# yshen47/SGAM_NeurIPS22

Measured on AMD Instinct MI355X. Metric: generated RGB-D frames/sec (256x256, GoogleEarth), higher is better.
Workload: dtype f32; 1 GPU; GoogleEarth-Infinite 256x256 inference loop (BASELINE configs[2]): forward-splat warp (N<=3) + VQGAN encode/quantise(4096)/decode + frame feedback, in-HBM frame store; frames_per_gpu=1110, scenes=1, parallelism=scene-parallel x1, launch=hip-graph replay of the VQGAN forward, f32_products=exact hi/lo fp16 split on the fp16 matrix cores, fp32 accumulate

## Files before the change

### include/sgam_hip.h

```cpp
#ifndef SGAM_HIP_H
#define SGAM_HIP_H

#include <stdint.h>

#ifdef __cplusplus
extern "C" {
#endif

#define SGAM_OK 0
#define SGAM_EINVAL (-1)
#define SGAM_EALIGN (-2)
#define SGAM_EWORKSPACE (-3)

int sgam_abi_version(void);
const char *sgam_build_info(void);
const char *sgam_build_commit(void);
const char *sgam_build_digest(void);

int sgam_prof_enable(int32_t on);
int sgam_prof_mark_empty(void *stream);
int32_t sgam_prof_count(void);
int sgam_prof_get(int32_t i, const char **kernel, const char **where, float *ms, double *flops, double *bytes);
int sgam_prof_get_shape(int32_t i, int32_t *mnks);

// ... 134 lines not shown
int64_t sgam_attn_block_f32x_workspace_bytes(int32_t n, int32_t C, int32_t B);
int sgam_attn_block_f32x(const float *x, int32_t ldx, const float *mean_rstd, const float *gamma, const float *beta, const void *wqkv_planes,
                         float wqkv_scale, const float *bqkv, int32_t n, int32_t C, int32_t B, float scale, const void *wp_planes,
                         float wp_scale, const float *bp, float *out, int32_t ldc, double *gn_partial, void *workspace,
                         int64_t workspace_bytes, void *stream);
int32_t sgam_attention_small_f32x_fits(int32_t n, int32_t C, int32_t B);
int sgam_attention_small_f32x(const float *q, const float *k, const float *v, int32_t ld, int32_t n, int32_t C, int32_t B, float scale,
                              float *out, int32_t ldo, void *stream);
int sgam_attention_small_h16(const void *q, const void *k, const void *v, int32_t ht, int32_t ld, int32_t n, int32_t C, int32_t B, float scale,
                             void *out, int32_t ldo, void *stream);
int sgam_groupnorm_table_from_partials(const double *partial, int32_t nchunk, const float *gamma, const float *beta,
                                       float *scale_shift, int32_t B, int32_t HW, int32_t C, int32_t groups, float eps, void *stream);
int sgam_pack_qkv_weight_h16(const float *w, void *w_frag, int32_t ht, int32_t C, void *stream);
int sgam_pack_weight_tp_h16(const float *w, void *w_frag, int32_t ht, int32_t rows, int32_t C, void *stream);
int sgam_attn_block_proj_h16(const void *x, int32_t ldx, const double *gn_partial, int32_t nchunk, const float *gamma, const float *beta,
                             float eps, const void *w_frag, const float *bias, int32_t ht, int32_t n, int32_t C, int32_t B, float scale,
                             const void *wp_frag, const float *bp, double *gn_partial_out, void *out, int32_t ldo, void *workspace,
                             int64_t workspace_bytes, void *stream);
int64_t sgam_attn_block_h16_workspace_bytes(int32_t n, int32_t C, int32_t B);
int sgam_attn_block_h16(const void *x, int32_t ldx, const double *gn_partial, int32_t nchunk, const float *gamma, const float *beta,
                        float eps, const void *w_frag, const float *bias, int32_t ht, int32_t n, int32_t C, int32_t B, float scale,
                        void *out, int32_t ldo, void *workspace, int64_t workspace_bytes, void *stream);

int sgam_row_sumsq_f32(const float *x, float *out, int32_t rows, int32_t cols, void *stream);
int64_t sgam_vq_workspace_bytes(int32_t T, int32_t D, int32_t n_e);
int sgam_vq_nearest_f32(const float *z, const float *codebook, const float *e_sq, float *dots,
                        int64_t *idx_out, float *zq_out, float *dist_out, int32_t T, int32_t D,
                        int32_t n_e, int32_t straight_through, void *workspace, int64_t workspace_bytes,
                        void *stream);
int sgam_vq_commit_loss_f32(const float *z, const float *codebook, const int64_t *idx, double *partial, float *loss,
                            int32_t T, int32_t D, int32_t n_e, float beta, void *stream);
int sgam_vq_gather_f32(const float *codebook, const int64_t *idx, float *out, int32_t T, int32_t D,
                       int32_t n_e, void *stream);
int sgam_vq_topk_f32(const float *dist, float *vals, int64_t *inds, int32_t T, int32_t n_e, int32_t k,
                     void *stream);
int sgam_vq_sample_topk_f32(const float *dist, const float *codebook, const uint8_t *mask, const int32_t *stream_id,
                            const uint64_t *call, uint64_t seed, float *vals, int64_t *inds, int64_t *idx_out,
                            float *zq_out, int32_t B, int32_t S, int32_t h, int32_t w, int32_t D, int32_t n_e,
                            int32_t k, int32_t mask_h, int32_t mask_w, int32_t per_token, float temperature,
                            void *stream);

int sgam_nchw_to_nhwc_f32(const float *x, float *y, int32_t B, int32_t C, int32_t HW, int32_t ldy,
                          void *stream);
int sgam_nhwc_to_nchw_f32(const float *x, float *y, int32_t B, int32_t C, int32_t HW, int32_t ldx,
                          void *stream);
int sgam_encode_head_f32(const float *x, const uint8_t *mask, const float *w, const float *bias,
                         float *y, int32_t B, int32_t HW, int32_t ldy, void *stream);

int sgam_forward_splat_f32(const float *src_feats, int64_t feat_cs, int64_t feat_ps,
                           const float *src_depths, const float *tgt_K, const float *src_Kinv,
                           const float *T, int32_t B, int32_t N, int32_t H, int32_t W,
                           const float *depth_range, int32_t dataset_norm, int32_t *winner,
                           float *merge_depths, float *merge_feats, uint8_t *extrap, float *x_out,
                           float *proj_feats, float *proj_depth, uint8_t *inb_mask, int32_t *pix_xy,
                           void *stream);
int sgam_forward_splat_srcs_f32(const float *const *src_feat_ptrs, const float *const *src_depth_ptrs, int64_t feat_cs,
                                int64_t feat_ps, const float *tgt_K, const float *src_Kinv, const float *T, int32_t B,
                                int32_t N, int32_t H, int32_t W, const float *depth_range, int32_t dataset_norm,
                                int32_t *winner, float *merge_depths, float *merge_feats, uint8_t *extrap, float *x_out,
                                float *proj_feats, float *proj_depth, uint8_t *inb_mask, int32_t *pix_xy, void *stream);

int64_t sgam_forward_splat_workspace_bytes(int32_t B, int32_t N, int32_t H, int32_t W);
int64_t sgam_forward_splat_workspace_zero_bytes(int32_t B, int32_t N, int32_t H, int32_t W);
int sgam_forward_splat_tiled_f32(const float *src_feats, int64_t feat_cs, int64_t feat_ps, const float *src_depths,
                                 const float *tgt_K, const float *src_Kinv, const float *T, int32_t B, int32_t N, int32_t H,
                                 int32_t W, const float *depth_range, int32_t dataset_norm, void *workspace,
// ... 142 lines not shown
```

### sgam_neurips22_amd/_lib.py

```python
import ctypes
import os

_PKG = os.path.dirname(os.path.abspath(__file__))
LIB_PATH = os.environ.get("SGAM_HIP_LIB") or os.path.join(_PKG, "lib", "libsgam_hip.so")

c_i32, c_i64, c_f32, c_vp = ctypes.c_int32, ctypes.c_int64, ctypes.c_float, ctypes.c_void_p


class ConvDesc(ctypes.Structure):
    _fields_ = [(n, c_i32) for n in (
        "B", "Hi", "Wi", "Cin", "Ho", "Wo", "N", "KH", "KW", "stride", "pad_t", "pad_l", "upsample2x",
        "lda", "ldb", "ldc", "ldr", "n_valid", "bias_per_row", "plan_bm", "plan_bn", "plan_ksplit")]


class TsdfGrid(ctypes.Structure):
    _fields_ = [("voxel_length", c_f32), ("sdf_trunc", c_f32), ("unit_base", c_i32 * 3), ("unit_dims", c_i32 * 3)]


class TsdfSrc(ctypes.Structure):
    _fields_ = [("depth", c_vp), ("rgb_u8", c_vp), ("cam2world", c_f32 * 16), ("world2cam", c_f32 * 16)]


ABI_VERSION = 10

# ... 129 lines not shown
                                              c_vp]),
    "sgam_softmax_rows_f32": (c_i32, [c_vp, c_i32, c_i32, c_i32, c_f32, c_vp]),
    "sgam_softmax_rows_blockdiag_f32": (c_i32, [c_vp, c_i32, c_i32, c_i32, c_f32, c_i32, c_vp]),
    "sgam_attention_f32x_workspace_bytes": (c_i64, [c_i32, c_i32]),
    "sgam_attention_f32x": (c_i32, [c_vp, c_vp, c_vp, c_i32, c_i32, c_i32, c_f32, c_vp, c_i32, c_vp, c_i64, c_vp]),
    "sgam_attention_h16_workspace_bytes": (c_i64, [c_i32, c_i32]),
    "sgam_attention_h16": (c_i32, [c_vp, c_vp, c_vp, c_i32, c_i32, c_i32, c_i32, c_f32, c_vp, c_i32, c_vp, c_i64, c_vp]),
    "sgam_attention_f32x_batched_workspace_bytes": (c_i64, [c_i32, c_i32, c_i32]),
    "sgam_attention_f32x_batched": (c_i32, [c_vp, c_vp, c_vp, c_i32, c_i32, c_i32, c_i32, c_f32, c_vp, c_i32, c_vp, c_i64, c_vp]),
    "sgam_attention_proj_f32x_batched": (c_i32, [c_vp, c_vp, c_vp, c_i32, c_i32, c_i32, c_i32, c_f32, c_vp, c_f32, c_vp, c_vp, c_i32, c_vp,
                                                 c_i32, c_vp, c_vp, c_i64, c_vp]),
    "sgam_attention_h16_batched_workspace_bytes": (c_i64, [c_i32, c_i32, c_i32]),
    "sgam_attention_h16_batched": (c_i32, [c_vp, c_vp, c_vp, c_i32, c_i32, c_i32, c_i32, c_i32, c_f32, c_vp, c_i32, c_vp, c_i64, c_vp]),
    "sgam_attn_block_f32x_workspace_bytes": (c_i64, [c_i32, c_i32, c_i32]),
    "sgam_attn_block_f32x": (c_i32, [c_vp, c_i32, c_vp, c_vp, c_vp, c_vp, c_f32, c_vp, c_i32, c_i32, c_i32, c_f32, c_vp, c_f32, c_vp, c_vp, c_i32,
                                     c_vp, c_vp, c_i64, c_vp]),
    "sgam_attention_small_f32x_fits": (c_i32, [c_i32, c_i32, c_i32]),
    "sgam_attention_small_f32x": (c_i32, [c_vp, c_vp, c_vp, c_i32, c_i32, c_i32, c_i32, c_f32, c_vp, c_i32, c_vp]),
    "sgam_attention_small_h16": (c_i32, [c_vp, c_vp, c_vp, c_i32, c_i32, c_i32, c_i32, c_i32, c_f32, c_vp, c_i32, c_vp]),
    "sgam_groupnorm_table_from_partials": (c_i32, [c_vp, c_i32, c_vp, c_vp, c_vp, c_i32, c_i32, c_i32, c_i32, c_f32, c_vp]),
    "sgam_pack_qkv_weight_h16": (c_i32, [c_vp, c_vp, c_i32, c_i32, c_vp]),
    "sgam_pack_weight_tp_h16": (c_i32, [c_vp, c_vp, c_i32, c_i32, c_i32, c_vp]),
    "sgam_attn_block_proj_h16": (c_i32, [c_vp, c_i32, c_vp, c_i32, c_vp, c_vp, c_f32, c_vp, c_vp, c_i32, c_i32, c_i32, c_i32, c_f32, c_vp, c_vp,
                                         c_vp, c_vp, c_i32, c_vp, c_i64, c_vp]),
    "sgam_attn_block_h16_workspace_bytes": (c_i64, [c_i32, c_i32, c_i32]),
    "sgam_attn_block_h16": (c_i32, [c_vp, c_i32, c_vp, c_i32, c_vp, c_vp, c_f32, c_vp, c_vp, c_i32, c_i32, c_i32, c_i32, c_f32, c_vp, c_i32,
                                    c_vp, c_i64, c_vp]),
    "sgam_row_sumsq_f32": (c_i32, [c_vp, c_vp, c_i32, c_i32, c_vp]),
    "sgam_vq_workspace_bytes": (c_i64, [c_i32, c_i32, c_i32]),
    "sgam_vq_nearest_f32": (c_i32, [c_vp, c_vp, c_vp, c_vp, c_vp, c_vp, c_vp, c_i32, c_i32, c_i32, c_i32, c_vp,
                                    c_i64, c_vp]),
    "sgam_vq_commit_loss_f32": (c_i32, [c_vp, c_vp, c_vp, c_vp, c_vp, c_i32, c_i32, c_i32, c_f32, c_vp]),
    "sgam_vq_gather_f32": (c_i32, [c_vp, c_vp, c_vp, c_i32, c_i32, c_i32, c_vp]),
    "sgam_vq_topk_f32": (c_i32, [c_vp, c_vp, c_vp, c_i32, c_i32, c_i32, c_vp]),
    "sgam_vq_sample_topk_f32": (c_i32, [c_vp, c_vp, c_vp, c_vp, c_vp, ctypes.c_uint64, c_vp, c_vp, c_vp, c_vp, c_i32, c_i32, c_i32, c_i32,
                                        c_i32, c_i32, c_i32, c_i32, c_i32, c_i32, c_f32, c_vp]),
    "sgam_nchw_to_nhwc_f32": (c_i32, [c_vp, c_vp, c_i32, c_i32, c_i32, c_i32, c_vp]),
    "sgam_nhwc_to_nchw_f32": (c_i32, [c_vp, c_vp, c_i32, c_i32, c_i32, c_i32, c_vp]),
    "sgam_encode_head_f32": (c_i32, [c_vp, c_vp, c_vp, c_vp, c_vp, c_i32, c_i32, c_i32, c_vp]),
    "sgam_forward_splat_f32": (c_i32, [c_vp, c_i64, c_i64, c_vp, c_vp, c_vp, c_vp, c_i32, c_i32, c_i32, c_i32,
                                       ctypes.POINTER(c_f32), c_i32, c_vp, c_vp, c_vp, c_vp, c_vp, c_vp, c_vp,
                                       c_vp, c_vp, c_vp]),
    "sgam_forward_splat_srcs_f32": (c_i32, [c_vp, c_vp, c_i64, c_i64, c_vp, c_vp, c_vp, c_i32, c_i32, c_i32, c_i32,
                                            ctypes.POINTER(c_f32), c_i32, c_vp, c_vp, c_vp, c_vp, c_vp, c_vp, c_vp,
                                            c_vp, c_vp, c_vp]),
    "sgam_forward_splat_workspace_bytes": (c_i64, [c_i32, c_i32, c_i32, c_i32]),
    "sgam_forward_splat_workspace_zero_bytes": (c_i64, [c_i32, c_i32, c_i32, c_i32]),
    "sgam_forward_splat_tiled_f32": (c_i32, [c_vp, c_i64, c_i64, c_vp, c_vp, c_vp, c_vp, c_i32, c_i32, c_i32, c_i32,
                                             ctypes.POINTER(c_f32), c_i32, c_vp, c_i64, c_vp, c_vp, c_vp, c_vp, c_vp, c_vp, c_vp]),
    "sgam_forward_splat_tiled_srcs_f32": (c_i32, [c_vp, c_vp, c_i64, c_i64, c_vp, c_vp, c_vp, c_i32, c_i32, c_i32, c_i32,
                                                  ctypes.POINTER(c_f32), c_i32, c_vp, c_i64, c_vp, c_vp, c_vp, c_vp, c_vp, c_vp,
                                                  c_vp]),
    "sgam_depth_normalise_f32": (c_i32, [c_vp, c_i32, c_vp, c_vp, c_i32, c_i64, c_vp]),
    "sgam_inverse_warp_f32": (c_i32, [c_vp, c_vp, c_vp, c_vp, c_vp, c_vp, c_i32, c_i32, c_i32, c_i32, c_vp, c_vp,
                                      c_vp]),
    "sgam_inverse_warp_srcs_f32": (c_i32, [c_vp, c_vp, c_i64, c_i64, c_vp, c_vp, c_vp, c_vp, c_i32, c_i32, c_i32, c_i32,
                                           c_vp, c_vp, c_vp]),
    "sgam_rgb_u8_to_f32": (c_i32, [c_vp, c_vp, c_vp, c_i64, c_vp]),
    "sgam_frame_feedback_f32": (c_i32, [c_vp, c_vp, c_i32, c_vp, c_vp, c_vp, c_i32, c_i32, c_vp]),
    "sgam_resize_lanczos_u8": (c_i32, [c_vp, c_i32, c_i32, c_i32, c_i32, c_i32, c_vp, c_vp, c_vp, c_i32, c_vp, c_vp, c_vp, c_i32,
                                       c_vp, c_vp, c_vp, c_vp]),
    "sgam_resize_nearest_f32": (c_i32, [c_vp, c_i32, c_i32, c_i32, c_i32, c_i32, c_vp, c_i32, c_f32, c_f32, c_vp, c_vp]),
}

_ERRORS = {-1: "SGAM_EINVAL (bad shape / unsupported size)", -2: "SGAM_EALIGN (pointer/stride alignment)",
           -3: "SGAM_EWORKSPACE (workspace missing or too small)"}
# ... 35 lines not shown
```

### sgam_neurips22_amd/csrc/vq.hip

```cpp
#include "sgam_common.h"

namespace {

__device__ __forceinline__ void argmin_combine(float &d, int &j, float od, int oj) {
    if (od < d || (od == d && oj < j)) {
        d = od;
        j = oj;
    }
}

__global__ __launch_bounds__(256) void vq_argmin_kernel(const float *__restrict__ z, const float *__restrict__ codebook,
                                                        const float *__restrict__ e_sq, const float *__restrict__ dots,
                                                        int64_t *__restrict__ idx_out, float *__restrict__ zq_out,
                                                        float *__restrict__ dist_out, int D, int n_e,
                                                        int straight_through) {
    const int t = blockIdx.x;
    const float *zr = z + (int64_t)t * D;
    __shared__ float red_f[4];
    __shared__ int red_i[4];
    __shared__ float bc_f;
    __shared__ int bc_i;

    float zz = 0.f;
    for (int c = threadIdx.x; c < D; c += 256) zz = __fmaf_rn(zr[c], zr[c], zz);
// ... 183 lines not shown
                                                                int T, int D, int n_e) {
    const int t = blockIdx.x * 4 + (threadIdx.x >> 6);
    if (t >= T) return;
    const int lane = threadIdx.x & 63;
    int64_t j = idx[t];
    j = j < 0 ? 0 : (j >= n_e ? n_e - 1 : j);
    double s = 0.0;
    for (int c = lane; c < D; c += 64) {
        const float d = __fsub_rn(codebook[j * D + c], z[(int64_t)t * D + c]);
        s += (double)d * (double)d;
    }
#pragma unroll
    for (int o = 32; o > 0; o >>= 1) s += __shfl_xor(s, o, 64);
    if (lane == 0) partial[t] = s;
}

__global__ __launch_bounds__(256) void vq_commit_fold_kernel(const double *__restrict__ partial, float *__restrict__ loss,
                                                             int T, int D, float beta) {
    __shared__ double red[256];
    double s = 0.0;
    for (int t = threadIdx.x; t < T; t += 256) s += partial[t];
    red[threadIdx.x] = s;
    __syncthreads();
    for (int o = 128; o > 0; o >>= 1) {
        if ((int)threadIdx.x < o) red[threadIdx.x] += red[threadIdx.x + o];
        __syncthreads();
    }
    if (threadIdx.x == 0) {
        const float m = (float)(red[0] / ((double)T * (double)D));
        loss[0] = __fadd_rn(m, __fmul_rn(beta, m));
    }
}

}

extern "C" int sgam_vq_commit_loss_f32(const float *z, const float *codebook, const int64_t *idx, double *partial,
                                       float *loss, int32_t T, int32_t D, int32_t n_e, float beta, void *stream) {
    if (!z || !codebook || !idx || !partial || !loss || T <= 0 || D <= 0 || n_e <= 0) return SGAM_EINVAL;
    SGAM_KLAUNCH(vq_commit_partial_kernel, dim3(sgam_cdiv(T, 4)), dim3(256), 0, sgam_stream(stream), z, codebook, idx,
                       partial, T, D, n_e);
    SGAM_LAUNCH_CHECK();
    SGAM_KLAUNCH(vq_commit_fold_kernel, dim3(1), dim3(256), 0, sgam_stream(stream), partial, loss, T, D, beta);
    SGAM_LAUNCH_CHECK();
    return SGAM_OK;
}

extern "C" int sgam_row_sumsq_f32(const float *x, float *out, int32_t rows, int32_t cols, void *stream) {
    if (!x || !out || rows <= 0 || cols <= 0) return SGAM_EINVAL;
    SGAM_KLAUNCH(row_sumsq_kernel, dim3(sgam_cdiv(rows, 4)), dim3(256), 0, sgam_stream(stream), x, out, rows, cols);
    SGAM_LAUNCH_CHECK();
    return SGAM_OK;
}

static sgam_conv_desc vq_dot_desc(int32_t T, int32_t D, int32_t n_e) {
    sgam_conv_desc d = {};
    d.B = 1; d.Hi = 1; d.Wi = T; d.Cin = D; d.Ho = 1; d.Wo = T; d.N = n_e;
    d.KH = 1; d.KW = 1; d.stride = 1; d.pad_t = 0; d.pad_l = 0; d.upsample2x = 0;
    d.lda = D; d.ldb = D; d.ldc = n_e; d.ldr = 0; d.n_valid = n_e; d.bias_per_row = 0;
    return d;
}

extern "C" int64_t sgam_vq_workspace_bytes(int32_t T, int32_t D, int32_t n_e) {
    if (T <= 0 || D <= 0 || D % 32 != 0 || n_e <= 0 || n_e % 64 != 0) return -1;
    const sgam_conv_desc d = vq_dot_desc(T, D, n_e);
    return sgam_conv2d_workspace_bytes(&d);
}
// ... 20 lines not shown
    SGAM_KLAUNCH(vq_gather_kernel, dim3(sgam_cdiv(total, 256)), dim3(256), 0, sgam_stream(stream), codebook, idx,
                       out, T, D, n_e);
    SGAM_LAUNCH_CHECK();
    return SGAM_OK;
}

extern "C" int sgam_vq_topk_f32(const float *dist, float *vals, int64_t *inds, int32_t T, int32_t n_e, int32_t k,
                                void *stream) {
    if (!dist || !vals || !inds || T <= 0 || n_e <= 0 || k <= 0 || k > 64 || k > n_e) return SGAM_EINVAL;
    SGAM_KLAUNCH(vq_topk_kernel, dim3(T), dim3(256), 0, sgam_stream(stream), dist, vals, inds, n_e, k);
    SGAM_LAUNCH_CHECK();
    return SGAM_OK;
}

extern "C" int sgam_vq_sample_topk_f32(const float *dist, const float *codebook, const uint8_t *mask, const int32_t *stream_id,
                                       const uint64_t *call, uint64_t seed, float *vals, int64_t *inds, int64_t *idx_out,
                                       float *zq_out, int32_t B, int32_t S, int32_t h, int32_t w, int32_t D, int32_t n_e,
                                       int32_t k, int32_t mask_h, int32_t mask_w, int32_t per_token, float temperature,
                                       void *stream) {
    if (!dist || !codebook || !stream_id || !call || !vals || !inds || !idx_out || !zq_out) return SGAM_EINVAL;
    if (B <= 0 || S <= 0 || h <= 0 || w <= 0 || D <= 0 || D % 4 != 0 || n_e <= 0 || k <= 0 || k > 32 || k > n_e) return SGAM_EINVAL;
    if (mask && (mask_h <= 0 || mask_w <= 0)) return SGAM_EINVAL;
    if (!(temperature > 0.f)) return SGAM_EINVAL;
    const int64_t T = (int64_t)h * w, rows = (int64_t)B * T, items = rows * S;
    if (rows > 0x7fffffff || items > 0x7fffffff || T * S > 0x7fffffff) return SGAM_EINVAL;
    SGAM_KLAUNCH(vq_topk_kernel, dim3((unsigned)rows), dim3(256), 0, sgam_stream(stream), dist, vals, inds, n_e, k);
    SGAM_LAUNCH_CHECK();
    SGAM_KLAUNCH(vq_sample_topk_kernel, dim3((unsigned)sgam_cdiv(items, 4)), dim3(256), 0, sgam_stream(stream), vals, inds,
                 codebook, mask, stream_id, reinterpret_cast<const uint32_t *>(call), (uint32_t)(seed & 0xffffffffu),
                 (uint32_t)(seed >> 32), idx_out, zq_out, B, S, h, w, D, n_e, k, mask_h, mask_w, per_token, temperature);
    SGAM_LAUNCH_CHECK();
    return SGAM_OK;
}
```

### sgam_neurips22_amd/generative_sensing_module/model.py

```python
import torch
import torch.nn as nn

from .. import ops
from ..point_rendering.warp import splat_to_model_input
from .modules.diffusionmodules.model import Conv2d, Decoder, Encoder
from .modules.vqvae.quantize import VectorQuantizer2 as VectorQuantizer


class VQModel(nn.Module):
    global_step = 0
    global_rank = 0

    def __init__(self, ddconfig, data_config, lossconfig, n_embed, embed_dim, phase=None, ckpt_path=None,
                 ignore_keys=['loss.discriminator'], image_key="image", colorize_nlabels=None, logdir=None,
                 use_extrapolation_mask=True, vq_step_threshold=0, monitor=None, remap=None, sane_index_shape=False,
                 online_kmeans_config=None, batch_size=None, depth_range=None):
        super().__init__()
        online_kmeans_config = online_kmeans_config or {}
        self.phase = phase
        self.online_kmeans_config = online_kmeans_config
        self.data_config = data_config
        self.logdir = logdir
        self.depth_range = depth_range
        self.n_embed = n_embed
# ... 96 lines not shown
        return _cm()

    def _forward_graphed(self, input, topk, extrapolation_mask, sample_number, flags):
        inplace = getattr(input, "_sgam_persistent", False) and (
            extrapolation_mask is None or getattr(extrapolation_mask, "_sgam_persistent", False))
        if self.compute_dtype == torch.float32 and ops.F32_MODE == "split":
            ops.range_flag(input.device)
        key = (tuple(input.shape), None if extrapolation_mask is None else tuple(extrapolation_mask.shape), topk,
               sample_number, flags, self.compute_dtype, str(input.device), ops.RANGE_FLAG_EPOCH,
               (input.data_ptr(), None if extrapolation_mask is None else extrapolation_mask.data_ptr()) if inplace else None)
        ent = self._graphs.get(key)
        if ent is None:
            sx = input if inplace else input.detach().clone()
            sm = None if extrapolation_mask is None else (extrapolation_mask if inplace else extrapolation_mask.detach().clone())
            side = torch.cuda.Stream()
            side.wait_stream(torch.cuda.current_stream())
            with torch.cuda.stream(side):
                for _ in range(2):
                    self._forward_guarded(sx, topk, sm, sample_number, flags)
            torch.cuda.current_stream().wait_stream(side)
            graph = torch.cuda.CUDAGraph()
            with torch.cuda.graph(graph):
                out = self._forward_eager(sx, topk, sm, sample_number, *flags)
            ent = self._graphs[key] = (graph, sx, sm, out)
        graph, sx, sm, out = ent
        if not inplace:
            sx.copy_(input)
            if sm is not None:
                sm.copy_(extrapolation_mask)
        graph.replay()
        return out

    def _encode_nhwc(self, x, extrapolation_mask):
        dt = self.compute_dtype
        if self.use_extrapolation_mask:
            h = ops.encode_head(x, extrapolation_mask, self.conv_in.weight, self.conv_in.bias, ld=32, dtype=dt)
        else:
            h = ops.cast(ops.nchw_to_nhwc(x, c_pad=32), dt)
        return self.quant_conv.forward_nhwc(self.encoder.forward_nhwc(h), out_dtype=torch.float32)

    def _decode_nhwc(self, quant_nhwc):
        q = ops.cast(quant_nhwc, self.compute_dtype)
        return self.decoder.forward_nhwc(self.post_quant_conv.forward_nhwc(q))

    def encode(self, x, topk=None, encoding_indices=None, extrapolation_mask=None, use_old=False, sample_number=1):
        pre = self._encode_nhwc(x, extrapolation_mask)
        if not self.use_vq():
            return ops.nhwc_to_nchw(pre)
        if topk is None:
            if encoding_indices is None:
                zq, idx, _ = self.quantize.quantize_nhwc(pre)
            else:
                B, h, w, D = pre.shape
                idx = encoding_indices.reshape(B, h, w)
                zq = ops.vq_gather(self.quantize._codebook()[0], idx).view(B, h, w, D)
            return ops.nhwc_to_nchw(zq), self.quantize.commit_loss_nhwc(pre, idx), (None, None, idx), ops.nhwc_to_nchw(pre)
        zqs, idx = self.quantize.sample_nhwc(pre, topk, sample_number, extrapolation_mask)
        quants = torch.stack([ops.nhwc_to_nchw(zqs[:, i].contiguous()) for i in range(zqs.shape[1])], 1)
        return quants, None, (None, None, idx), ops.nhwc_to_nchw(pre)

    def decode(self, quant):
        return ops.nhwc_to_nchw(self._decode_nhwc(ops.nchw_to_nhwc(quant)))

    def forward(self, input, topk=None, extrapolation_mask=None, sample_number=1, get_codebook_count=False,
                get_pre_quantized_feature=False, get_quantized_feature=False):
        flags = (bool(get_codebook_count), bool(get_pre_quantized_feature), bool(get_quantized_feature))
        ds = self.quantize.device_sampler
        host_rng = self.quantize.consume_host_rng if topk == 1 else ds is None
        replay_safe = topk is None or not host_rng
        sampling = ds is not None and topk is not None and topk > 1 and input.is_cuda and self.use_vq()
        if sampling:
            ds.begin(input.shape[0], input.device)
        try:
            if self.use_hip_graph and not getattr(self, "_graph_bypass", False) and replay_safe and input.is_cuda \
                    and not torch.is_grad_enabled():
                return self._forward_graphed(input, topk, extrapolation_mask, sample_number, flags)
            return self._forward_guarded(input, topk, extrapolation_mask, sample_number, flags)
        finally:
            if sampling:
                ds.end()

    range_check = "sync"

    def _guard_active(self, input):
        return (self.range_check == "sync" and input.is_cuda and self.compute_dtype == torch.float32
                and ops.F32_MODE == "split" and not torch.cuda.is_current_stream_capturing())

    def _forward_guarded(self, input, topk, extrapolation_mask, sample_number, flags):
        guard = self._guard_active(input)
        if guard:
            ops.range_flag(input.device)
            rng = torch.get_rng_state() if (topk is not None and topk > 1 and self.quantize.device_sampler is None) else None
        out = self._forward_eager(input, topk, extrapolation_mask, sample_number, *flags)
        if guard and ops.f32x_range_tripped():
            import warnings
            warnings.warn("sgam split-fp32 path: an activation left fp16's range (|x| >= 65520) and produced a non-finite "
                          "value; recomputing on the fp32-in MFMA path and switching SGAM_F32_MODE to 'mfma'", RuntimeWarning)
            ops.set_f32_mode("mfma")
            self._graphs = {}
            if rng is not None:
                torch.set_rng_state(rng)
            out = self._forward_eager(input, topk, extrapolation_mask, sample_number, *flags)
        return out

    def _forward_eager(self, input, topk=None, extrapolation_mask=None, sample_number=1, get_codebook_count=False,
                       get_pre_quantized_feature=False, get_quantized_feature=False):
        pre = self._encode_nhwc(input, extrapolation_mask)
        if not self.use_vq():
            dec = ops.nhwc_to_nchw(self._decode_nhwc(pre))
            return dec, torch.tensor(0).to(dec.device), ops.nhwc_to_nchw(pre)
        want_q = get_quantized_feature
        diff = None
        if topk is None:
            zq, idx, _ = self.quantize.quantize_nhwc(pre)
            diff = self.quantize.commit_loss_nhwc(pre, idx)
            decs = ops.nhwc_to_nchw(self._decode_nhwc(zq))
            quants = ops.nhwc_to_nchw(zq) if want_q else None
        else:
            zqs, idx = self.quantize.sample_nhwc(pre, topk, sample_number, extrapolation_mask)
            zs = [zqs[:, i].contiguous() for i in range(sample_number)]
            decs = [ops.nhwc_to_nchw(self._decode_nhwc(z))[None] for z in zs]
            quants = zqs.permute(0, 1, 4, 2, 3) if want_q else None
        res = [decs, diff]
        if get_codebook_count:
            res.append(idx)
        if get_pre_quantized_feature:
            res.append(pre.permute(0, 3, 1, 2) if not torch.is_grad_enabled() else ops.nhwc_to_nchw(pre))
        if get_quantized_feature:
            res.append(quants)
        return res

    learning_rate = 4.5e-6

    def init_loss(self):
        if getattr(self, "loss", None) is None:
            from ..config import instantiate_from_config
            if not self.lossconfig or not self.lossconfig.get("target"):
                raise ops.SgamHipError("VQModel: lossconfig has no `target` — nothing to train against")
            self.loss = instantiate_from_config(self.lossconfig).to(self.device)
        return self.loss

    def _trainer_for_step(self):
        tr = getattr(self, "_trainer", None)
        if tr is None:
            from .. import training
            loss = self.init_loss()
# ... 82 lines not shown
```

### sgam_neurips22_amd/ops.py

```python
import ctypes
import os

import torch

from . import _lib
from ._lib import ConvDesc, SgamHipError, check

from ._opscore import *
from ._opscore import _c, _dense_nhwc, _f32c, _need_cuda, _p, _stream


F32_MODE = os.environ.get("SGAM_F32_MODE", "split")
PANEL_GEMM = os.environ.get("SGAM_PANEL_GEMM", "1") == "1"
PANEL_MIN_WGS = int(os.environ.get("SGAM_PANEL_MIN_WGS", "1"))
FUSE_GN_STATS = os.environ.get("SGAM_FUSE_GN_STATS", "1") == "1"
FUSE_GN_APPLY = os.environ.get("SGAM_FUSE_GN_APPLY", "1") == "1"


_RANGE_FLAGS = {}
_RANGE_FLAG_ACTIVE = None


def _dev_index(device):
    d = torch.device(device)
    if d.type != "cuda":
        raise SgamHipError(f"range_flag: {d} is not a HIP device")
    return torch.cuda.current_device() if d.index is None else d.index


def range_flag(device):
    global _RANGE_FLAG_ACTIVE, RANGE_FLAG_EPOCH
    i = _dev_index(device)
    t = _RANGE_FLAGS.get(i)
    if t is None:
        t = _RANGE_FLAGS[i] = torch.zeros((1,), device=torch.device("cuda", i), dtype=torch.int32)
    if _RANGE_FLAG_ACTIVE != i:
        check(_lib.load().sgam_f32x_set_range_flag(_p(t)), "sgam_f32x_set_range_flag")
        _RANGE_FLAG_ACTIVE = i
        RANGE_FLAG_EPOCH += 1
    return t


RANGE_FLAG_EPOCH = 0


def f32x_range_tripped(reset=True, device=None):
    i = _RANGE_FLAG_ACTIVE if device is None else _dev_index(device)
# ... 770 lines not shown
```

### sgam_neurips22_amd/ops_aux.py

```python
import ctypes

import torch

from . import _lib
from ._lib import SgamHipError, check
from ._opscore import *
from ._opscore import _c, _dense_nhwc, _f32c, _need_cuda, _p, _stream

def _kernel_name(kernel, where):
    import re
    name = kernel.strip().strip("()").replace(" ", "")
    m = re.search(r"\[([^\]]*)\]\s*$", where or "")
    if m and "<" in name:
        sub = dict(kv.split(" = ") for kv in m.group(1).split(", ") if " = " in kv)
        head, args = name.split("<", 1)
        args = [sub.get(a, a) for a in args.rstrip(">").split(",")]
        name = f"{head}<{','.join(args)}>"
    return name


def kernel_timeline(fn, empty_brackets=32):
    lib = _lib.load()
    torch.cuda.synchronize()
    check(lib.sgam_prof_enable(1), "sgam_prof_enable")
# ... 82 lines not shown
    dots = torch.empty((T, n_e), device=z.device, dtype=torch.float32)
    idx = torch.empty((T,), device=z.device, dtype=torch.int64)
    zq = torch.empty((T, D), device=z.device, dtype=torch.float32) if want_zq else None
    dist = torch.empty((T, n_e), device=z.device, dtype=torch.float32) if want_dist else None
    ws_bytes = lib.sgam_vq_workspace_bytes(T, D, n_e)
    if ws_bytes < 0:
        raise SgamHipError(f"sgam_vq: unsupported shape T={T} D={D} n_e={n_e}")
    ws = torch.empty((ws_bytes,), device=z.device, dtype=torch.uint8) if ws_bytes else None
    check(lib.sgam_vq_nearest_f32(_p(z), _p(codebook), _p(e_sq), _p(dots), _p(idx), _p(zq), _p(dist), T, D, n_e,
                                  int(straight_through), _p(ws), ws_bytes, _stream()), "sgam_vq_nearest_f32")
    return idx, zq, dist


def vq_commit_loss(z_tokens, codebook, idx, beta):
    _need_cuda(z_tokens, codebook, idx)
    z = _f32c(z_tokens)
    T, D = z.shape
    partial = torch.empty((T,), device=z.device, dtype=torch.float64)
    loss = torch.empty((1,), device=z.device, dtype=torch.float32)
    idx = idx.reshape(-1)
    check(_lib.load().sgam_vq_commit_loss_f32(_p(z), _p(codebook), _p(idx), _p(partial), _p(loss), T, D, codebook.shape[0],
                                              float(beta), _stream()), "sgam_vq_commit_loss_f32")
    return loss[0]


def vq_gather(codebook, idx):
    _need_cuda(codebook, idx)
    idx = idx.reshape(-1).to(torch.int64).contiguous()
    T, D = idx.numel(), codebook.shape[1]
    out = torch.empty((T, D), device=codebook.device, dtype=torch.float32)
    check(_lib.load().sgam_vq_gather_f32(_p(codebook), _p(idx), _p(out), T, D, codebook.shape[0], _stream()),
          "sgam_vq_gather_f32")
    return out


def vq_topk(dist, k):
    _need_cuda(dist)
    T, n_e = dist.shape
    vals = torch.empty((T, k), device=dist.device, dtype=torch.float32)
    inds = torch.empty((T, k), device=dist.device, dtype=torch.int64)
    check(_lib.load().sgam_vq_topk_f32(_p(dist), _p(vals), _p(inds), T, n_e, k, _stream()), "sgam_vq_topk_f32")
    return vals, inds


def vq_sample_topk(dist, codebook, topk, sample_number, hw, stream_id, call, seed=0, mask=None, per_token=False,
                   temperature=1.0):
    _need_cuda(dist, codebook, stream_id, call)
    h, w = int(hw[0]), int(hw[1])
    rows, n_e = dist.shape
    D = codebook.shape[1]
    if rows % (h * w) != 0 or not dist.is_contiguous() or dist.dtype != torch.float32:
        raise SgamHipError(f"vq_sample_topk: dist {tuple(dist.shape)} is not a dense fp32 (B*{h}*{w}, n_e) matrix")
    B, S, k = rows // (h * w), int(sample_number), int(topk)
    if stream_id.dtype != torch.int32 or stream_id.numel() != B or not stream_id.is_contiguous():
        raise SgamHipError(f"vq_sample_topk: stream_id must be a contiguous int32 tensor of {B} entries")
    if call.numel() * call.element_size() < 8 or call.data_ptr() % 8 != 0:
        raise SgamHipError("vq_sample_topk: call must be an 8-byte aligned device buffer of at least 8 bytes")
    m, mH, mW = None, 0, 0
    if mask is not None:
        _need_cuda(mask)
        mH, mW = mask.shape[-2:]
        m = mask.reshape(B, mH, mW)
        if m.dtype == torch.bool and m.is_contiguous():
            m = m.view(torch.uint8)
        else:
            m = (m != 0).to(torch.uint8).contiguous()
# ... 64 lines not shown
```

Measured before the change: 368.2 frames/s.

## Fuse quant_conv, VQ nearest-code search, and post_quant_conv into two kernels

Adds a fused VQ bottleneck path. A front kernel does the quant_conv 1x1 GEMM using the hi/lo fp16 split on MFMA, then computes codebook distances in f32 MFMA and a per-tile argmin. A back kernel reduces the argmin, gathers the code vectors, computes the commit-loss partials and runs the post_quant_conv GEMM. This removes several separate launches and the HBM round trips for z, the dot matrix and zq between quant_conv, VQ and post_quant_conv. In exchange, the quant_conv GEMM is recomputed in every codebook tile block (n_e/128 times), and the path only applies to specific shapes.

```diff
diff --git a/include/sgam_hip.h b/include/sgam_hip.h
--- a/include/sgam_hip.h
+++ b/include/sgam_hip.h
@@ -190,6 +190,13 @@
                             int32_t T, int32_t D, int32_t n_e, float beta, void *stream);
 int sgam_vq_gather_f32(const float *codebook, const int64_t *idx, float *out, int32_t T, int32_t D,
                        int32_t n_e, void *stream);
+int32_t sgam_vq_bottleneck_f32x_fits(int32_t T, int32_t HW, int32_t C, int32_t D, int32_t n_e);
+int64_t sgam_vq_bottleneck_f32x_workspace_bytes(int32_t T, int32_t HW, int32_t C, int32_t D, int32_t n_e);
+int sgam_vq_bottleneck_f32x(const float *h, int32_t ldh, const void *wq_planes, float wq_scale, const float *bq,
+                            const float *codebook, const float *e_sq, const void *wp_planes, float wp_scale, const float *bp,
+                            float *z_out, int64_t *idx_out, float *zq_out, double *partial, float *loss, float *out, int32_t T,
+                            int32_t HW, int32_t C, int32_t D, int32_t n_e, int32_t straight_through, float beta, void *workspace,
+                            int64_t workspace_bytes, void *stream);
 int sgam_vq_topk_f32(const float *dist, float *vals, int64_t *inds, int32_t T, int32_t n_e, int32_t k,
                      void *stream);
 int sgam_vq_sample_topk_f32(const float *dist, const float *codebook, const uint8_t *mask, const int32_t *stream_id,
diff --git a/sgam_neurips22_amd/_lib.py b/sgam_neurips22_amd/_lib.py
--- a/sgam_neurips22_amd/_lib.py
+++ b/sgam_neurips22_amd/_lib.py
@@ -185,6 +185,10 @@
                                     c_i64, c_vp]),
     "sgam_vq_commit_loss_f32": (c_i32, [c_vp, c_vp, c_vp, c_vp, c_vp, c_i32, c_i32, c_i32, c_f32, c_vp]),
     "sgam_vq_gather_f32": (c_i32, [c_vp, c_vp, c_vp, c_i32, c_i32, c_i32, c_vp]),
+    "sgam_vq_bottleneck_f32x_fits": (c_i32, [c_i32, c_i32, c_i32, c_i32, c_i32]),
+    "sgam_vq_bottleneck_f32x_workspace_bytes": (c_i64, [c_i32, c_i32, c_i32, c_i32, c_i32]),
+    "sgam_vq_bottleneck_f32x": (c_i32, [c_vp, c_i32, c_vp, c_f32, c_vp, c_vp, c_vp, c_vp, c_f32, c_vp, c_vp, c_vp, c_vp, c_vp, c_vp, c_vp,
+                                        c_i32, c_i32, c_i32, c_i32, c_i32, c_i32, c_f32, c_vp, c_i64, c_vp]),
     "sgam_vq_topk_f32": (c_i32, [c_vp, c_vp, c_vp, c_i32, c_i32, c_i32, c_vp]),
     "sgam_vq_sample_topk_f32": (c_i32, [c_vp, c_vp, c_vp, c_vp, c_vp, ctypes.c_uint64, c_vp, c_vp, c_vp, c_vp, c_i32, c_i32, c_i32, c_i32,
                                         c_i32, c_i32, c_i32, c_i32, c_i32, c_i32, c_f32, c_vp]),
diff --git a/sgam_neurips22_amd/csrc/vq.hip b/sgam_neurips22_amd/csrc/vq.hip
--- a/sgam_neurips22_amd/csrc/vq.hip
+++ b/sgam_neurips22_amd/csrc/vq.hip
@@ -239,6 +239,285 @@
     }
 }
 
+
+typedef unsigned int u32x4 __attribute__((ext_vector_type(4)));
+typedef _Float16 f16x8 __attribute__((ext_vector_type(8)));
+
+constexpr int VF_ROWS = 32, VF_CODES = 128, VF_K = 256;
+constexpr int VF_LDK = VF_K + 8;
+constexpr int VF_LDZ = VF_K + 4;
+constexpr int VF_SMEM = 2 * VF_ROWS * VF_LDK * 2;
+static_assert(VF_ROWS * VF_LDZ * 4 <= VF_SMEM, "the z tile must fit in the panel's LDS");
+
+__device__ __forceinline__ f32x16 vq_mfma16(u32x4 a, u32x4 b, f32x16 c) {
+    return __builtin_amdgcn_mfma_f32_32x32x16_f16(__builtin_bit_cast(f16x8, a), __builtin_bit_cast(f16x8, b), c, 0, 0, 0);
+}
+
+__device__ __forceinline__ void vq_stage_split(unsigned short *sA, int row, int c4, f32x4 v) {
+    unsigned hi[2], lo[2];
+#pragma unroll
+    for (int e = 0; e < 2; ++e) {
+        const float a0 = v[2 * e], a1 = v[2 * e + 1];
+        const _Float16 h0 = (_Float16)a0, h1 = (_Float16)a1;
+        const _Float16 l0 = (_Float16)(a0 - (float)h0), l1 = (_Float16)(a1 - (float)h1);
+        hi[e] = (unsigned)__builtin_bit_cast(unsigned short, h0) | ((unsigned)__builtin_bit_cast(unsigned short, h1) << 16);
+        lo[e] = (unsigned)__builtin_bit_cast(unsigned short, l0) | ((unsigned)__builtin_bit_cast(unsigned short, l1) << 16);
+    }
+    *reinterpret_cast<unsigned long long *>(sA + row * VF_LDK + c4) = (unsigned long long)hi[0] | ((unsigned long long)hi[1] << 32);
+    *reinterpret_cast<unsigned long long *>(sA + (VF_ROWS + row) * VF_LDK + c4) = (unsigned long long)lo[0] | ((unsigned long long)lo[1] << 32);
+}
+
+__device__ __forceinline__ void vq_panel_mma(const unsigned short *sA, const unsigned short *__restrict__ w, int wave, int lane,
+                                             f32x16 (&acc)[2]) {
+    constexpr int WD = 4, KS = VF_K / 16, SLABS = VF_K / 32;
+    const int lr = lane & 31, lh = lane >> 5;
+    const unsigned short *wt[2] = {w + (int64_t)(wave * 2) * SLABS * 2048, w + (int64_t)(wave * 2 + 1) * SLABS * 2048};
+    u32x4 wh[2][WD], wl[2][WD];
+    auto wfrag = [&](int j, int kstep, u32x4 &hi, u32x4 &lo) {
+        const unsigned short *q = wt[j] + (kstep >> 1) * 2048 + (((kstep & 1) * 2 + lh) * 32 + lr) * 8;
+        hi = *reinterpret_cast<const u32x4 *>(q);
+        lo = *reinterpret_cast<const u32x4 *>(q + 1024);
+    };
+#pragma unroll
+    for (int j = 0; j < 2; ++j)
+#pragma unroll
+        for (int t = 0; t < WD; ++t) wfrag(j, t, wh[j][t], wl[j][t]);
+#pragma unroll
+    for (int j = 0; j < 2; ++j)
+#pragma unroll
+        for (int e = 0; e < 16; ++e) acc[j][e] = 0.f;
+    __syncthreads();
+#pragma unroll
+    for (int t = 0; t < KS; ++t) {
+        u32x4 bh[2], bl[2];
+#pragma unroll
+        for (int j = 0; j < 2; ++j) {
+            bh[j] = wh[j][t % WD], bl[j] = wl[j][t % WD];
+            if (t + WD < KS) wfrag(j, t + WD, wh[j][t % WD], wl[j][t % WD]);
+        }
+        __builtin_amdgcn_sched_barrier(0);
+        const u32x4 ah = *reinterpret_cast<const u32x4 *>(sA + lr * VF_LDK + t * 16 + lh * 8);
+        const u32x4 al = *reinterpret_cast<const u32x4 *>(sA + (VF_ROWS + lr) * VF_LDK + t * 16 + lh * 8);
+#pragma unroll
+        for (int j = 0; j < 2; ++j) {
+            acc[j] = vq_mfma16(ah, bh[j], acc[j]);
+            acc[j] = vq_mfma16(ah, bl[j], acc[j]);
+            acc[j] = vq_mfma16(al, bh[j], acc[j]);
+        }
+    }
+}
+
+struct VqFusedParams {
+    const float *h;
+    const unsigned short *wq;
+    const float *bq;
+    const float *codebook;
+    const float *e_sq;
+    const unsigned short *wp;
+    const float *bp;
+    float *z;
+    float *pair_d;
+    int *pair_j;
+    int64_t *idx;
+    float *zq;
+    double *partial;
+    float *out;
+    int32_t *range_flag;
+    float inv_wq, inv_wp;
+    int ldh, T, n_e, tiles, straight_through;
+};
+
+template <int SPLITS>
+__global__ __launch_bounds__(256) void vq_front_f32x_kernel(const VqFusedParams p) {
+    __shared__ __attribute__((aligned(16))) unsigned char smem[VF_SMEM];
+    __shared__ float s_zz[VF_ROWS];
+    __shared__ float s_rd[4][VF_ROWS];
+    __shared__ int s_rj[4][VF_ROWS];
+    unsigned short *sA = reinterpret_cast<unsigned short *>(smem);
+    float *sZ = reinterpret_cast<float *>(smem);
+    const int tid = threadIdx.x, lane = tid & 63, wave = tid >> 6, lr = lane & 31, lh = lane >> 5;
+    const int m0 = blockIdx.x * VF_ROWS, tile = blockIdx.y;
+    const int code = tile * VF_CODES + wave * 32 + lr;
+
+    f32x4 cb[VF_K / 8];
+    {
+        const f32x4 *er = reinterpret_cast<const f32x4 *>(p.codebook + (int64_t)code * VF_K) + lh;
+#pragma unroll
+        for (int q = 0; q < VF_K / 8; ++q) cb[q] = er[2 * q];
+    }
+    const float esq = p.e_sq[code];
+
+    const int prow = tid >> 6, pc4 = (tid & 63) * 4;
+    {
+        f32x4 xr[8];
+#pragma unroll
+        for (int it = 0; it < 8; ++it)
+            xr[it] = *reinterpret_cast<const f32x4 *>(p.h + (int64_t)(m0 + prow + 4 * it) * p.ldh + pc4);
+#pragma unroll
+        for (int it = 0; it < 8; ++it) vq_stage_split(sA, prow + 4 * it, pc4, xr[it]);
+    }
+    f32x16 acc[2];
+    vq_panel_mma(sA, p.wq, wave, lane, acc);
+    __syncthreads();
+    {
+        float gs = 0.f;
+#pragma unroll
+        for (int j = 0; j < 2; ++j) {
+            const int n = wave * 64 + j * 32 + lr;
+            const float bias = p.bq ? p.bq[n] : 0.f;
+#pragma unroll
+            for (int e = 0; e < 16; ++e) {
+                const int row = 8 * (e >> 2) + 4 * lh + (e & 3);
+                const float v = __fmaf_rn(acc[j][e], p.inv_wq, bias);
+                sZ[row * VF_LDZ + n] = v;
+                if (tile == 0) p.z[(int64_t)(m0 + row) * VF_K + n] = v;
+                gs += v;
+            }
+        }
+        if (tile == 0 && p.range_flag && sgam_not_finite(gs)) atomicOr(p.range_flag, 1);
+    }
+    __syncthreads();
+
+#pragma unroll
+    for (int r = 0; r < 8; ++r) {
+        const int row = wave * 8 + r;
+        float q[4];
+#pragma unroll
+        for (int w = 0; w < 4; ++w) {
+            const float v = sZ[row * VF_LDZ + w * 64 + lane];
+            q[w] = sgam_wave_sum(__fmaf_rn(v, v, 0.f));
+        }
+        if (lane == 0) s_zz[row] = (q[0] + q[1]) + (q[2] + q[3]);
+    }
+
+    f32x16 dot;
+    {
+        constexpr int SLABS_PER = (VF_K / 32) / SPLITS;
+        const float *zr = sZ + lr * VF_LDZ + lh * 4;
+#pragma unroll
+        for (int z = 0; z < SPLITS; ++z) {
+            f32x16 a;
+#pragma unroll
+            for (int e = 0; e < 16; ++e) a[e] = 0.f;
+#pragma unroll
+            for (int q = z * SLABS_PER * 4; q < (z + 1) * SLABS_PER * 4; ++q) {
+                const f32x4 af = *reinterpret_cast<const f32x4 *>(zr + q * 8);
+#pragma unroll
+                for (int s = 0; s < 4; ++s) a = __builtin_amdgcn_mfma_f32_32x32x2f32(af[s], cb[q][s], a, 0, 0, 0);
+            }
+#pragma unroll
+            for (int e = 0; e < 16; ++e) {
+                const float v = (a[e] + 0.f) + 0.f;
+                dot[e] = z == 0 ? v : dot[e] + v;
+            }
+        }
+    }
+    __syncthreads();
+
+#pragma unroll
+    for (int e = 0; e < 16; ++e) {
+        const int row = 8 * (e >> 2) + 4 * lh + (e & 3);
+        float d = __fsub_rn(__fadd_rn(s_zz[row], esq), __fmul_rn(2.0f, dot[e]));
+        int j = code;
+        if (!(d < INFINITY)) {
+            d = INFINITY;
+            j = 0x7fffffff;
+        }
+#pragma unroll
+        for (int o = 16; o > 0; o >>= 1) {
+            const float od = __shfl_xor(d, o, 64);
+            const int oj = __shfl_xor(j, o, 64);
+            argmin_combine(d, j, od, oj);
+        }
+        if (lr == 0) {
+            s_rd[wave][row] = d;
+            s_rj[wave][row] = j;
+        }
+    }
+    __syncthreads();
+    if (tid < VF_ROWS) {
+        float d = s_rd[0][tid];
+        int j = s_rj[0][tid];
+        for (int w = 1; w < 4; ++w) argmin_combine(d, j, s_rd[w][tid], s_rj[w][tid]);
+        p.pair_d[(int64_t)(m0 + tid) * p.tiles + tile] = d;
+        p.pair_j[(int64_t)(m0 + tid) * p.tiles + tile] = j;
+    }
+}
+
+__global__ __launch_bounds__(256) void vq_back_f32x_kernel(const VqFusedParams p) {
+    __shared__ __attribute__((aligned(16))) unsigned short sA[2 * VF_ROWS * VF_LDK];
+    __shared__ int s_idx[VF_ROWS];
+    const int tid = threadIdx.x, lane = tid & 63, wave = tid >> 6, lr = lane & 31, lh = lane >> 5;
+    const int m0 = blockIdx.x * VF_ROWS;
+
+    {
+        const int row = tid >> 3, sub = tid & 7;
+        float d = INFINITY;
+        int j = 0x7fffffff;
+        for (int t = sub; t < p.tiles; t += 8)
+            argmin_combine(d, j, p.pair_d[(int64_t)(m0 + row) * p.tiles + t], p.pair_j[(int64_t)(m0 + row) * p.tiles + t]);
+#pragma unroll
+        for (int o = 4; o > 0; o >>= 1) {
+            const float od = __shfl_xor(d, o, 64);
+            const int oj = __shfl_xor(j, o, 64);
+            argmin_combine(d, j, od, oj);
+        }
+        if (sub == 0) {
+            if (j == 0x7fffffff) j = 0;
+            s_idx[row] = j;
+            p.idx[m0 + row] = (int64_t)j;
+        }
+    }
+    __syncthreads();
+
+    const int prow = tid >> 6, pc4 = (tid & 63) * 4;
+#pragma unroll
+    for (int it = 0; it < 8; ++it) {
+        const int row = prow + 4 * it;
+        f32x4 v = *reinterpret_cast<const f32x4 *>(p.codebook + (int64_t)s_idx[row] * VF_K + pc4);
+        if (p.straight_through) {
+            const f32x4 zv = *reinterpret_cast<const f32x4 *>(p.z + (int64_t)(m0 + row) * VF_K + pc4);
+#pragma unroll
+            for (int e = 0; e < 4; ++e) v[e] = __fadd_rn(zv[e], __fsub_rn(v[e], zv[e]));
+        }
+        *reinterpret_cast<f32x4 *>(p.zq + (int64_t)(m0 + row) * VF_K + pc4) = v;
+        vq_stage_split(sA, row, pc4, v);
+    }
+
+    if (p.partial) {
+#pragma unroll 1
+        for (int r = 0; r < 8; ++r) {
+            const int row = wave * 8 + r, t = m0 + row;
+            const int64_t j = s_idx[row];
+            double s = 0.0;
+            for (int c = lane; c < VF_K; c += 64) {
+                const float d = __fsub_rn(p.codebook[j * VF_K + c], p.z[(int64_t)t * VF_K + c]);
+                s += (double)d * (double)d;
+            }
+#pragma unroll
+            for (int o = 32; o > 0; o >>= 1) s += __shfl_xor(s, o, 64);
+            if (lane == 0) p.partial[t] = s;
+        }
+    }
+
+    f32x16 acc[2];
+    vq_panel_mma(sA, p.wp, wave, lane, acc);
+    float gs = 0.f;
+#pragma unroll
+    for (int j = 0; j < 2; ++j) {
+        const int n = wave * 64 + j * 32 + lr;
+        const float bias = p.bp ? p.bp[n] : 0.f;
+#pragma unroll
+        for (int e = 0; e < 16; ++e) {
+            const int row = 8 * (e >> 2) + 4 * lh + (e & 3);
+            const float v = __fmaf_rn(acc[j][e], p.inv_wp, bias);
+            p.out[(int64_t)(m0 + row) * VF_K + n] = v;
+            gs += v;
+        }
+    }
+    if (p.range_flag && sgam_not_finite(gs)) atomicOr(p.range_flag, 1);
+}
+
 }
 
 extern "C" int sgam_vq_commit_loss_f32(const float *z, const float *codebook, const int64_t *idx, double *partial,
@@ -325,3 +604,65 @@
     SGAM_LAUNCH_CHECK();
     return SGAM_OK;
 }
+
+static int vq_bottleneck_splits(int32_t T, int32_t HW, int32_t C, int32_t D, int32_t n_e) {
+    if (T <= 0 || T % 64 != 0 || C != VF_K || D != VF_K || n_e <= 0 || n_e % VF_CODES != 0) return 0;
+    if ((int64_t)T * (n_e / VF_CODES) > 0x7fffffff || n_e / VF_CODES > 65535) return 0;
+    if (HW <= 0 || sgam_gemm_gn_f32x_fits(T, D, C, HW) != 1 || sgam_gemm_gn_f32x_fits(T, C, D, HW) != 1) return 0;
+    const sgam_conv_desc d = vq_dot_desc(T, D, n_e);
+    int32_t ks = 0;
+    if (sgam_conv2d_plan(&d, nullptr, nullptr, &ks) != SGAM_OK) return 0;
+    return (ks == 1 || ks == 2) ? ks : 0;
+}
+
+extern "C" int32_t sgam_vq_bottleneck_f32x_fits(int32_t T, int32_t HW, int32_t C, int32_t D, int32_t n_e) {
+    return vq_bottleneck_splits(T, HW, C, D, n_e) > 0 ? 1 : 0;
+}
+
+extern "C" int64_t sgam_vq_bottleneck_f32x_workspace_bytes(int32_t T, int32_t HW, int32_t C, int32_t D, int32_t n_e) {
+    if (vq_bottleneck_splits(T, HW, C, D, n_e) == 0) return -1;
+    return (int64_t)T * (n_e / VF_CODES) * 8;
+}
+
+extern "C" int sgam_vq_bottleneck_f32x(const float *h, int32_t ldh, const void *wq_planes, float wq_scale, const float *bq,
+                                       const float *codebook, const float *e_sq, const void *wp_planes, float wp_scale,
+                                       const float *bp, float *z_out, int64_t *idx_out, float *zq_out, double *partial, float *loss,
+                                       float *out, int32_t T, int32_t HW, int32_t C, int32_t D, int32_t n_e, int32_t straight_through, float beta,
+                                       void *workspace, int64_t workspace_bytes, void *stream) {
+    if (!h || !wq_planes || !codebook || !e_sq || !wp_planes || !z_out || !idx_out || !zq_out || !out) return SGAM_EINVAL;
+    if ((partial == nullptr) != (loss == nullptr) || !(wq_scale > 0.f) || !(wp_scale > 0.f)) return SGAM_EINVAL;
+    const int splits = vq_bottleneck_splits(T, HW, C, D, n_e);
+    if (splits == 0 || ldh < C) return SGAM_EINVAL;
+    if (!sgam_aligned16(h) || ldh % 4 || !sgam_aligned16(wq_planes) || !sgam_aligned16(wp_planes) || !sgam_aligned16(codebook) ||
+        !sgam_aligned16(z_out) || !sgam_aligned16(zq_out))
+        return SGAM_EALIGN;
+    const int tiles = n_e / VF_CODES;
+    const int64_t need = (int64_t)T * tiles * 8;
+    if (!workspace || workspace_bytes < need || !sgam_aligned16(workspace)) return SGAM_EWORKSPACE;
+    VqFusedParams p;
+    p.h = h; p.wq = (const unsigned short *)wq_planes; p.bq = bq; p.codebook = codebook; p.e_sq = e_sq;
+    p.wp = (const unsigned short *)wp_planes; p.bp = bp; p.z = z_out;
+    p.pair_d = (float *)workspace; p.pair_j = (int *)workspace + (int64_t)T * tiles;
+    p.idx = idx_out; p.zq = zq_out; p.partial = partial; p.out = out; p.range_flag = sgam_i_range_flag;
+    p.inv_wq = 1.0f / wq_scale; p.inv_wp = 1.0f / wp_scale;
+    p.ldh = ldh; p.T = T; p.n_e = n_e; p.tiles = tiles; p.straight_through = straight_through;
+    hipStream_t s = sgam_stream(stream);
+    const dim3 grid(T / VF_ROWS, tiles);
+    if (sgam_i_prof_on) sgam_i_prof_shape(T, n_e, D, splits);
+    if (sgam_i_prof_on)
+        sgam_i_prof_work(2.0 * T * (double)D * C + 2.0 * T * (double)n_e * D,
+                         4.0 * ((double)T * C + (double)D * C + (double)n_e * D + (double)T * D + 2.0 * T * tiles));
+    if (splits == 1) SGAM_KLAUNCH((vq_front_f32x_kernel<1>), grid, dim3(256), 0, s, p);
+    else SGAM_KLAUNCH((vq_front_f32x_kernel<2>), grid, dim3(256), 0, s, p);
+    SGAM_LAUNCH_CHECK();
+    if (sgam_i_prof_on) sgam_i_prof_shape(T, C, D, 1);
+    if (sgam_i_prof_on)
+        sgam_i_prof_work(2.0 * T * (double)C * D, 4.0 * (2.0 * T * tiles + 3.0 * T * D + (double)C * D + (double)T * C));
+    SGAM_KLAUNCH(vq_back_f32x_kernel, dim3(T / VF_ROWS), dim3(256), 0, s, p);
+    SGAM_LAUNCH_CHECK();
+    if (loss) {
+        SGAM_KLAUNCH(vq_commit_fold_kernel, dim3(1), dim3(256), 0, s, partial, loss, T, D, beta);
+        SGAM_LAUNCH_CHECK();
+    }
+    return SGAM_OK;
+}
diff --git a/sgam_neurips22_amd/generative_sensing_module/model.py b/sgam_neurips22_amd/generative_sensing_module/model.py
--- a/sgam_neurips22_amd/generative_sensing_module/model.py
+++ b/sgam_neurips22_amd/generative_sensing_module/model.py
@@ -152,16 +152,35 @@
         return out
 
     def _encode_nhwc(self, x, extrapolation_mask):
+        return self.quant_conv.forward_nhwc(self._encoder_nhwc(x, extrapolation_mask), out_dtype=torch.float32)
+
+    def _encoder_nhwc(self, x, extrapolation_mask):
         dt = self.compute_dtype
         if self.use_extrapolation_mask:
             h = ops.encode_head(x, extrapolation_mask, self.conv_in.weight, self.conv_in.bias, ld=32, dtype=dt)
         else:
             h = ops.cast(ops.nchw_to_nhwc(x, c_pad=32), dt)
-        return self.quant_conv.forward_nhwc(self.encoder.forward_nhwc(h), out_dtype=torch.float32)
+        return self.encoder.forward_nhwc(h)
 
     def _decode_nhwc(self, quant_nhwc):
         q = ops.cast(quant_nhwc, self.compute_dtype)
         return self.decoder.forward_nhwc(self.post_quant_conv.forward_nhwc(q))
+
+    def _bottleneck_fused(self, henc, topk, sample_number):
+        if not (self.use_vq() and henc.is_cuda and henc.dtype == torch.float32 and self.compute_dtype == torch.float32
+                and ops.F32_MODE == "split" and ops.PANEL_GEMM and ops.PANEL_MIN_WGS <= 1 and ops.VQ_BOTTLENECK_FUSED
+                and not torch.is_grad_enabled()):
+            return None
+        if not (topk is None or (topk == 1 and sample_number == 1 and not self.quantize.consume_host_rng)):
+            return None
+        B, hh, ww, C = henc.shape
+        if not ops.vq_bottleneck_fits(B * hh * ww, hh * ww, C, self.quantize.e_dim, self.quantize.n_e):
+            return None
+        wq, bq = self.quant_conv._packed(torch.float32)
+        wp, bp = self.post_quant_conv._packed(torch.float32)
+        if not (isinstance(wq, ops.SplitWeight) and isinstance(wp, ops.SplitWeight)):
+            return None
+        return wq, bq, wp, bp
 
     def encode(self, x, topk=None, encoding_indices=None, extrapolation_mask=None, use_old=False, sample_number=1):
         pre = self._encode_nhwc(x, extrapolation_mask)
@@ -225,13 +244,33 @@
 
     def _forward_eager(self, input, topk=None, extrapolation_mask=None, sample_number=1, get_codebook_count=False,
                        get_pre_quantized_feature=False, get_quantized_feature=False):
-        pre = self._encode_nhwc(input, extrapolation_mask)
+        want_q = get_quantized_feature
+        diff = None
+        henc = self._encoder_nhwc(input, extrapolation_mask)
+        fused = self._bottleneck_fused(henc, topk, sample_number)
+        if fused is not None:
+            wq, bq, wp, bp = fused
+            cb, cb_sq = self.quantize._codebook()
+            B, hh, ww, _ = henc.shape
+            pre, idx, zq, diff, pq = ops.vq_bottleneck(henc, wq, bq, cb, cb_sq, wp, bp, straight_through=topk is None,
+                                                       beta=self.quantize.beta if topk is None else None)
+            dec = ops.nhwc_to_nchw(self.decoder.forward_nhwc(pq))
+            if topk is None:
+                zq, idx = zq.view(B, hh, ww, -1), idx.view(B, hh, ww)
+                decs = dec
+                quants = ops.nhwc_to_nchw(zq) if want_q else None
+            else:
+                zqs, idx = zq.view(B, 1, hh, ww, -1), idx.view(B, 1, hh, ww)
+                decs = [dec[None]]
+                quants = zqs.permute(0, 1, 4, 2, 3) if want_q else None
+        else:
+            pre = self.quant_conv.forward_nhwc(henc, out_dtype=torch.float32)
         if not self.use_vq():
             dec = ops.nhwc_to_nchw(self._decode_nhwc(pre))
             return dec, torch.tensor(0).to(dec.device), ops.nhwc_to_nchw(pre)
-        want_q = get_quantized_feature
-        diff = None
-        if topk is None:
+        if fused is not None:
+            pass
+        elif topk is None:
             zq, idx, _ = self.quantize.quantize_nhwc(pre)
             diff = self.quantize.commit_loss_nhwc(pre, idx)
             decs = ops.nhwc_to_nchw(self._decode_nhwc(zq))
diff --git a/sgam_neurips22_amd/ops.py b/sgam_neurips22_amd/ops.py
--- a/sgam_neurips22_amd/ops.py
+++ b/sgam_neurips22_amd/ops.py
@@ -13,6 +13,7 @@
 F32_MODE = os.environ.get("SGAM_F32_MODE", "split")
 PANEL_GEMM = os.environ.get("SGAM_PANEL_GEMM", "1") == "1"
 PANEL_MIN_WGS = int(os.environ.get("SGAM_PANEL_MIN_WGS", "1"))
+VQ_BOTTLENECK_FUSED = os.environ.get("SGAM_VQ_BOTTLENECK_FUSED", "1") != "0"
 FUSE_GN_STATS = os.environ.get("SGAM_FUSE_GN_STATS", "1") == "1"
 FUSE_GN_APPLY = os.environ.get("SGAM_FUSE_GN_APPLY", "1") == "1"
 
diff --git a/sgam_neurips22_amd/ops_aux.py b/sgam_neurips22_amd/ops_aux.py
--- a/sgam_neurips22_amd/ops_aux.py
+++ b/sgam_neurips22_amd/ops_aux.py
@@ -138,6 +138,35 @@
     check(_lib.load().sgam_vq_gather_f32(_p(codebook), _p(idx), _p(out), T, D, codebook.shape[0], _stream()),
           "sgam_vq_gather_f32")
     return out
+
+
+def vq_bottleneck_fits(T, HW, C, D, n_e):
+    return _lib.load().sgam_vq_bottleneck_f32x_fits(int(T), int(HW), int(C), int(D), int(n_e)) == 1
+
+
+def vq_bottleneck(h, wq, bq, codebook, e_sq, wp, bp, straight_through=True, beta=None):
+    _need_cuda(h, codebook, e_sq)
+    h = _c(h)
+    B, hh, ww, ld = h.shape
+    T, HW, n_e, D = B * hh * ww, hh * ww, codebook.shape[0], codebook.shape[1]
+    C = wq.shape[1]
+    lib = _lib.load()
+    ws_bytes = lib.sgam_vq_bottleneck_f32x_workspace_bytes(T, HW, C, D, n_e)
+    if ws_bytes < 0 or h.dtype != torch.float32 or wq.shape[0] != D or tuple(wp.shape) != (C, D):
+        raise SgamHipError(f"sgam_vq_bottleneck_f32x: unsupported shape T={T} HW={HW} C={C} D={D} n_e={n_e}")
+    dev = h.device
+    ws = torch.empty((ws_bytes,), device=dev, dtype=torch.uint8)
+    z = torch.empty((B, hh, ww, D), device=dev, dtype=torch.float32)
+    idx = torch.empty((T,), device=dev, dtype=torch.int64)
+    zq = torch.empty((T, D), device=dev, dtype=torch.float32)
+    out = torch.empty((B, hh, ww, C), device=dev, dtype=torch.float32)
+    partial = torch.empty((T,), device=dev, dtype=torch.float64) if beta is not None else None
+    loss = torch.empty((1,), device=dev, dtype=torch.float32) if beta is not None else None
+    check(lib.sgam_vq_bottleneck_f32x(_p(h), ld, _p(wq.planes), float(wq.scale), _p(bq), _p(codebook), _p(e_sq),
+                                      _p(wp.planes), float(wp.scale), _p(bp), _p(z), _p(idx), _p(zq), _p(partial), _p(loss), _p(out),
+                                      T, HW, C, D, n_e, int(straight_through), float(beta or 0.0), _p(ws), ws_bytes, _stream()),
+          "sgam_vq_bottleneck_f32x")
+    return z, idx, zq, (loss[0] if loss is not None else None), out
 
 
 def vq_topk(dist, k):
```

Measured after the change: 368.2 frames/s. Within noise of the previous version (-0.0%).
